# Illumina/strelka

Measured on AMD Instinct MI355X. Metric: candidate-alignment scoring cells/s (read bases x candidate alignments; Strelka2 has no pair-HMM, SURVEY.md section 0) + germline loci/s + 40x WGS-like germline wall-clock (e2e) + 110x/40x somatic wall-clock (e2e_somatic), higher is better.
Workload: dtype f64; 1 GPU; germline chr20-style synthetic (BASELINE.json configs[1]).  Headline: scoreCandidateAlignment as one function -- per GPU per step 65536 reads of 150 bp x 87.9 candidate alignments each (5-7 candidate indels around them), from the candidate alignments the device search left (PCal) to one double each: one kernel (F5: the walk of each alignment's path + the terms of its bases, penalties and clips).  ; read_len=150

## Files before the change

strelka_amd/csrc/read_enumerate.hip:

```cpp

#include "sk_common.h"

#include "align_entry.h"
#include "read_enumerate.h"

#include <algorithm>
#include <chrono>
#include <climits>
#include <cstdio>
#include <cstdlib>
#include <cstring>
#include <vector>

using namespace skcore;

int sk_score_alignments_launch_hostleg(const sk_align_batch* b, double* dev_out_lnp, void* hip_stream);

namespace
{

static_assert(sizeof(PFrame) % 4 == 0 && sizeof(PCal) % 4 == 0, "frames move through LDS as 32-bit words");


struct EnumArgs
// ... 365 lines not shown
    const char* ref;
    int32_t ref_offset, ref_len;
    int32_t n_reads, n_cals;
    const PCal* pool;
    const int32_t* list;
    int32_t* status;
    const int64_t* read_off;
    const uint8_t* read_code;
    const int32_t* cal_off;
    int32_t* win_begin;
    int32_t* win_end;
    int32_t* ins_lo;
    int32_t* ins_hi;
    uint8_t* n_seg8;
    int32_t* win_len;
    int32_t* hap_len;
    int32_t* n_ins;
    int16_t* ins_idx;
    int32_t* ins_off;
    int32_t* n_ops;
    const int64_t* hap_off;
    PCal* cals;
    uint8_t* hap_code;
    const int64_t* op_off;
    sk_score_op* ops;
    uint32_t* entries;
    uint32_t* evmask;
    int32_t evmask_words, max_read_len;
    uint8_t* colmat;
    const int64_t* colmat_off;
    uint32_t* addmask;
    int32_t* ref_outside;
    int32_t n_cals_on_device;
};
enum { INS_CAP = Caps::K + 2 };

__device__ inline int read_of_cal(const FlatArgs& a, const int c)
{
    int lo = 0, hi = a.n_reads;
    while (hi - lo > 1) {
        const int mid = (lo + hi) >> 1;
        if (a.cal_off[mid] <= c) lo = mid; else hi = mid;
    }
    return lo;
}

__global__ __launch_bounds__(256) void pool_bounds_kernel(const FlatArgs a)
{
    const int n_cals = a.n_cals_on_device ? a.cal_off[a.n_reads] : a.n_cals;
    for (int c = blockIdx.x * blockDim.x + threadIdx.x; c < n_cals; c += gridDim.x * blockDim.x) {
    const int r = read_of_cal(a, c);
    const PCal& cal = a.pool[a.list[c]];
    a.n_seg8[c] = uint8_t(min(int(cal.n_seg), 255));
    int32_t wb = INT_MAX, we = INT_MIN, pos = cal.pos;
    for (int i = 0; i < cal.n_seg; ++i) {
        const PSeg s = cal.path[i];
        if (seg_align_match(s.type)) {
            wb = min(wb, pos);
            we = max(we, pos + int32_t(s.length));
            pos += int32_t(s.length);
        } else if (s.type == SK_SEG_DELETE || s.type == SK_SEG_SKIP) {
            pos += int32_t(s.length);
        }
    }
    if (wb <= we) {
        atomicMin(&a.win_begin[r], wb);
        atomicMax(&a.win_end[r], we);
    }
    int lo = INT_MAX, hi = INT_MIN;
    auto add = [&](const int t) {
        if (t < 0 || a.job.tab[t].ins_len == 0) return;
        lo = min(lo, t);
        hi = max(hi, t);
    };
    for (int i = 0; i < cal.n_indels; ++i) add(cal.indels[i]);
    add(cal.lead);
    add(cal.trail);
    if (lo <= hi) {
        atomicMin(&a.ins_lo[r], lo);
        atomicMax(&a.ins_hi[r], hi);
    }
    }
}

__global__ __launch_bounds__(64) void pool_layout_kernel(const FlatArgs a)
{
    const int r = blockIdx.x * blockDim.x + threadIdx.x;
    if (r >= a.n_reads) return;
    const int nc = a.cal_off[r + 1] - a.cal_off[r];
    a.n_ins[r] = 0;
    a.win_len[r] = 0;
    a.hap_len[r] = 0;
    if (nc == 0) return;
    int32_t wb = a.win_begin[r], we = a.win_end[r];
    if (wb > we) wb = we = 0;
    a.win_begin[r] = wb;
    int32_t len = we - wb;
    a.win_len[r] = len;
    int16_t* idx = a.ins_idx + size_t(r) * INS_CAP;
    int32_t* off = a.ins_off + size_t(r) * INS_CAP;
    int n = 0;
    for (int t = a.ins_lo[r]; t <= a.ins_hi[r]; ++t) {
        const uint32_t il = a.job.tab[t].ins_len;
        if (il == 0) continue;
        if (n >= INS_CAP) {
            a.status[r] = ST_OVERFLOW;
            n = 0;
            break;
        }
        idx[n] = int16_t(t);
        off[n] = len;
        len += int32_t(il);
        ++n;
    }
    a.n_ins[r] = n;
    a.hap_len[r] = max(len, 1);
}

__device__ int matching_indel(const PJob& j, const PCal& c, const int32_t ref_head_pos, const unsigned del_len, const unsigned ins_len,
                              const int ends_first, const int ends_second, const int path_index)
{
    if (path_index < ends_first) return c.lead;
    if (path_index > ends_second) return c.trail;
    int found = -1;
    for (int k = 0; k < c.n_indels; ++k) {
        const PIndel& ci = j.tab[c.indels[k]];
        if (ci.pos == ref_head_pos && (ci.type == SK_INDEL_INDEL || ci.type == SK_INDEL_MISMATCH) && ci.del == del_len &&
            ci.ins_len == ins_len) {
            if (found >= 0) return -2;
            found = c.indels[k];
        } else if (ci.pos > ref_head_pos) {
            break;
        }
    }
    return found >= 0 ? found : -2;
}

struct NoOpSink
{
    __device__ __forceinline__ void operator()(uint8_t, uint32_t, int32_t, bool) const {}
};

template <bool WRITE, typename SINK = NoOpSink>
__device__ int flatten_cal(const FlatArgs& a, const int r, const PCal& c, const int32_t read_len, sk_score_op* ops, SINK&& sink = SINK())
{
    const int aps = c.n_seg;
    const int32_t win_begin = a.win_begin[r];
    const int n_ins = a.n_ins[r];
    const int16_t* ins_idx = a.ins_idx + size_t(r) * INS_CAP;
// ... 157 lines not shown
    const int c0 = blockIdx.x * blockDim.x;
    const int c = c0 + lane;
    const int nc = min(64, a.n_cals - c0);
    const int src_k = (lane < nc) ? a.list[c0 + lane] : 0;
    for (int k = 0; k < nc; ++k) {
        const uint32_t* __restrict__ src = reinterpret_cast<const uint32_t*>(a.pool + __shfl(src_k, k));
        uint32_t* __restrict__ dst = reinterpret_cast<uint32_t*>(a.cals + (c0 + k));
        for (int j = lane; j < REC_DW; j += 64) {
            const uint32_t v = src[j];
            s_cal[k * REC_STRIDE + j] = v;
            dst[j] = v;
        }
    }
    __syncthreads();
    if (c >= a.n_cals) return;
    const int r = read_of_cal(a, c);
    const PCal& cal = *reinterpret_cast<const PCal*>(s_cal + lane * REC_STRIDE);
    if (a.status[r] != ST_OK) return;
    (void)flatten_cal<true>(a, r, cal, int32_t(a.read_off[r + 1] - a.read_off[r]), a.ops + a.op_off[c]);
    for (int i = 0; i < cal.n_indels; ++i) (void)job_cand(a.job, cal.indels[i]);
    if (cal.lead >= 0) (void)job_cand(a.job, cal.lead);
    if (cal.trail >= 0) (void)job_cand(a.job, cal.trail);
}

constexpr int F5_MAX_READ = 256;
constexpr int ONE_WAIT_MAX_READS = 16384;
constexpr int F5_MAX_POOL = 768;
#ifndef F5_SORT
#define F5_SORT 1
#endif
constexpr int F5_TAB = 32;

static_assert(F5_TAB <= 64, "the table copy is a lane an entry");

struct FusedScoreArgs
{
    FlatArgs f;
    const uint8_t* read_qual;
    const SkTables* tab;
    double* scores;
    unsigned* err;
    int32_t* n_unhandled;
    int32_t write_cals;
    unsigned long long* dbg;
    unsigned* queue;
};

constexpr int F5_SEGS = 16, F5_INDELS = 8;
constexpr int F5_SLOT = (F5_SEGS + 1) | 1;
__device__ __forceinline__ int f5_ent_word(const int k) { return k; }
constexpr int F5_ROW = 3;

struct F5Tab
{
    int32_t pos;
    uint32_t del, ins_len;
    uint32_t type_cand;
    int32_t ins_at;
};

template <int MAXR>
struct F5Lds
{
    uint8_t read[MAXR + 12];
    uint8_t hap[F5_MAX_POOL + 12];
    double row[(MAXR + 8) * F5_ROW];
// ... 67 lines not shown
        }
    }
    int pi = 0, n_ent = 0;
    int32_t pos = 0, ref_head_pos = c.pos();
    unsigned npen = 0;
    for (;;) {
        const bool live = pi < aps && !bad;
        if (!__any(live)) break;
        const int sh = 4 * (pi & 15);
        const unsigned ty = unsigned(types >> sh) & 15u, ln = seg_len(pi & 15);
        const uint64_t not_run = ~((I4 | D4) >> sh) & N1;
        const int run4 = not_run ? __builtin_ctzll(not_run) : 64;
        const uint64_t run_set = (run4 >= 64) ? ~0ull : ((1ull << run4) - 1ull);
        const bool is_swap = live && ((I4 >> sh) & run_set) != 0ull && ((D4 >> sh) & run_set) != 0ull;
        const bool is_match = (ty == SK_SEG_MATCH || ty == SK_SEG_SEQ_MATCH), is_clip = (ty == SK_SEG_SOFT_CLIP);
        const bool is_indel_seg = is_swap || ty == SK_SEG_SEQ_MISMATCH || ty == SK_SEG_INSERT || ty == SK_SEG_DELETE;
        unsigned del_len = (ty == SK_SEG_INSERT) ? 0u : ln, ins_len = (ty == SK_SEG_DELETE) ? 0u : ln;
        int n_seg = 1;
        unsigned read_step = (is_match || ty == SK_SEG_SEQ_MISMATCH || ty == SK_SEG_INSERT || is_clip) ? ln : 0u;
        unsigned ref_step = (is_match || ty == SK_SEG_SEQ_MISMATCH || ty == SK_SEG_DELETE || ty == SK_SEG_SKIP) ? ln : 0u;
        if (is_swap) {
            n_seg = run4 >> 2;
            del_len = ins_len = 0;
            for (int k = 0; k < n_seg; ++k) {
                const unsigned l = seg_len((pi + k) & 15);
                if ((I4 >> (4 * ((pi + k) & 15))) & 1ull) ins_len += l;
                else del_len += l;
            }
            read_step = ins_len;
            ref_step = del_len;
        }
        const unsigned asked = (del_len << 16) | ins_len;
        const bool askable = del_len < 0xffffu && ins_len < 0xffffu;
        int k_found = 0, n_found = 0;
        bool open = true;
#pragma unroll
        for (int k = 0; k < F5_INDELS; ++k) {
            if (k < ni_wave) {
                const bool m = open && k_pos[k] == ref_head_pos && k_pack[k] == asked;
                k_found = m ? k : k_found;
                n_found += m ? 1 : 0;
                open = open && (m || k_pos[k] <= ref_head_pos);
            }
        }
        int key = (n_found == 1) ? c.indel(k_found) : -2;
        key = (pi < ends_first) ? c.lead() : (pi > ends_second) ? c.trail() : key;
        const bool key_ok = key >= 0;
        const F5Tab te = S.tab[(key_ok ? key : tab_lo) - tab_lo];
        const bool indel_ok = live && is_indel_seg && key_ok;
        if (indel_ok && consulted) consulted[key] = 1;
        const bool pen = is_indel_seg && (te.type_cand >> 8) == 0u;
        const int32_t head = (pi < ends_first) ? int32_t(te.ins_len) - int32_t(ln) : 0;
        const bool ins_bases = is_indel_seg && ins_len > 0u;
        const bool ins_ok = ins_len <= 0xffffu && head >= 0 && uint32_t(head) + ins_len <= te.ins_len && te.ins_at >= 0;
        const bool bases = ins_bases || is_match;
        const int32_t src = ins_bases ? te.ins_at + head : ref_head_pos - win_begin;
        const unsigned len = ins_bases ? ins_len : ln;
        const bool known = is_indel_seg || is_match || is_clip || ty == SK_SEG_SKIP || ty == SK_SEG_HARD_CLIP;
        bool fail = !known || (is_indel_seg && (!key_ok || !askable)) || (ins_bases && !ins_ok);
        const bool entry = (bases || (is_clip && !is_indel_seg)) && len > 0u;
        if (entry) {
            fail = fail || pos + int32_t(len) > L || (bases && (src < 0 || int64_t(src) + int64_t(len) > int64_t(P)));
            const int hidx = bases ? int(src) - pos : 0;
            fail = fail || n_ent > F5_SEGS || npen > 4u || hidx < -256 || hidx > 3839;
            if (live && !fail) myslot[f5_ent_word(n_ent)] = unsigned(pos) | (npen << 9) | (bases ? 0u : 1u << 15) | (unsigned(hidx + 256) << 16);
        }
        if (live) {
            bad = fail;
            n_ent += entry ? 1 : 0;
            npen = entry ? (pen ? 1u : 0u) : npen + (pen ? 1u : 0u);
            pos += int32_t(read_step);
            ref_head_pos += int32_t(ref_step);
            pi += n_seg;
        }
    }
    if (!has) return 0;
    if (bad || pos != L || n_ent > F5_SEGS || npen > 4u) return -1;
    myslot[f5_ent_word(n_ent)] = unsigned(L) | (npen << 9) | (256u << 16);
    return n_ent + 1;
}

template <typename LDS>
__device__ __forceinline__ double f5_sum(LDS& S, const uint32_t* const myslot, const int n_ent, const double ln_noncand, const double ln_quarter)
{
    double lnp = 0.0;
    const unsigned char* rows = reinterpret_cast<const unsigned char*>(S.row);
    int e = 0, p = 0, stop = 0, hidx = 0;
    uint32_t cur = myslot[f5_ent_word(0)], nxt = myslot[f5_ent_word(1)];
    auto next_op = [&]() -> bool {
// ... 42 lines not shown
                uint32_t pm = uint32_t(past >> (32 * h));
                __asm__("" : "+v"(pm));
                sel[h] = (B10 & ~pm & x) | (~B10 & pm);
                __asm__("" : "+v"(sel[h]));
            }
            const unsigned base = __umul24(unsigned(8 * F5_ROW), unsigned(p));
            double v[8];
#pragma unroll
            for (int u = 0; u < 8; ++u) {
                const unsigned at = base + unsigned(8 * F5_ROW * u) + ((sel[u >> 2] >> (8 * (u & 3))) & 0xffu);
                v[u] = *reinterpret_cast<const double*>(rows + at);
            }
#pragma unroll
            for (int u = 0; u < 8; ++u) lnp = __dadd_rn(lnp, v[u]);
            p += mm;
        }
        if (next_op()) break;
    }
    return lnp;
}

__device__ __forceinline__ void f5_wave_sync()
{
    __builtin_amdgcn_fence(__ATOMIC_RELEASE, "workgroup");
    __builtin_amdgcn_wave_barrier();
    __builtin_amdgcn_fence(__ATOMIC_ACQUIRE, "workgroup");
}

template <int MAXR, bool TIMING>
__device__ __forceinline__ void f5_read(const FusedScoreArgs& fa, const int r, F5Lds<MAXR>& S)
{
    auto now = [&]() -> unsigned long long { return TIMING ? (unsigned long long)clock64() : 0ull; };
    const FlatArgs& a = fa.f;
    const int lane = threadIdx.x & 63;
    const int c0 = a.cal_off[r], c1 = a.cal_off[r + 1];
    const int ncr = c1 - c0;
    if (ncr == 0 || a.status[r] != ST_OK) return;
    unsigned long long stamp[8];
    stamp[0] = now();
    const unsigned long long wall0 = TIMING ? (unsigned long long)wall_clock64() : 0ull;
    for (int i = 1; i < 8; ++i) stamp[i] = 0;
    const int64_t ro = a.read_off[r];
    const int32_t L = int32_t(a.read_off[r + 1] - ro);
    const int32_t P = a.hap_len[r];
    if (L > MAXR || P > F5_MAX_POOL) {
        if (lane == 0) atomicAdd(fa.n_unhandled, 1);
        return;
    }
    const int32_t win_begin = a.win_begin[r];
    const int n_ins = a.n_ins[r];
    int my_ins_idx = -1;
    int32_t my_ins_off = 0;
    {
        const int16_t* idx = a.ins_idx + size_t(r) * INS_CAP;
        const int32_t* off = a.ins_off + size_t(r) * INS_CAP;
        int32_t my_ins_len = 0;
        uint32_t my_ins_src = 0;
        if (lane < n_ins) {
            const int t_idx = idx[lane];
            my_ins_idx = t_idx;
            my_ins_off = off[lane];
            my_ins_len = int32_t(a.job.tab[t_idx].ins_len);
            my_ins_src = a.job.tab[t_idx].ins_off;
        }
        const int32_t win_len = a.win_len[r];
        for (int32_t i = lane; i < P + 8; i += 64) {
            uint8_t v = SK_BAM_ANY;
            if (i < win_len) {
                const int32_t p = win_begin + i;
                const bool outside = (p < a.ref_offset || p >= a.ref_offset + a.ref_len);
                if (outside && a.ref_outside) atomicAdd(a.ref_outside, 1);
                v = outside ? uint8_t(SK_BAM_ANY) : code_of(a.ref[p - a.ref_offset]);
            }
            S.hap[i] = v;
        }
        f5_wave_sync();
        for (int k = 0; k < n_ins; ++k) {
            const int32_t o = __builtin_amdgcn_readlane(my_ins_off, k), n = __builtin_amdgcn_readlane(my_ins_len, k);
            const uint32_t src = uint32_t(__builtin_amdgcn_readlane(int(my_ins_src), k));
            for (int32_t i = lane; i < n; i += 64)
                if (o + i < P) S.hap[o + i] = code_of(a.ins_pool[src + uint32_t(i)]);
        }
        const SkTables* __restrict__ T = fa.tab;
        for (int32_t i = lane; i < L + 12; i += 64) {
            unsigned q = 0;
            uint8_t code = SK_BAM_ANY;
            if (i < L) {
                code = a.read_code[ro + i];
                q = fa.read_qual[ro + i];
                if (q > 70u) {
                    atomicOr(fa.err, unsigned(SK_DEVERR_QSCORE));
                    q = 70u;
                }
            }
            S.read[i] = code & 15u;
            if (i < L + 8) {
                const unsigned c = code & 15u;
                const bool adds = i < L && c != 15u;
                const double agree = adds ? T->q2lncompe[q] : 0.0;
                S.row[F5_ROW * i] = agree;
                S.row[F5_ROW * i + 1] = 0.0;
                S.row[F5_ROW * i + 2] = !adds ? 0.0 : (c == 0u) ? agree : T->q2mis[q];
            }
        }
    }
    const double ln_quarter = fa.tab->ln_quarter, ln_noncand = fa.tab->ln_noncand;

    uint8_t* const order = S.hap + ((P + 8 + 3) & ~3);
    const bool sorted_order = (F5_SORT != 0) && ncr > 64 && ncr <= 256 && ((P + 8 + 3) & ~3) + ncr <= int(sizeof(S.hap));
    if (sorted_order) {
        int seg_of[4];
#pragma unroll
        for (int k = 0; k < 4; ++k) {
            const int j = lane + 64 * k;
            seg_of[k] = (j < ncr) ? int(a.n_seg8[c0 + j]) : -1;
            seg_of[k] = min(seg_of[k], F5_SEGS + 1);
        }
        unsigned present = 0;
#pragma unroll
        for (int k = 0; k < 4; ++k) present |= (seg_of[k] >= 0) ? (1u << seg_of[k]) : 0u;
#pragma unroll
        for (int d = 32; d >= 1; d >>= 1) present |= unsigned(__shfl_xor(int(present), d));
        present = unsigned(__builtin_amdgcn_readfirstlane(int(present)));
        int at = 0;
        while (present != 0u) {
            const int v = 31 - __builtin_clz(present);
            present &= ~(1u << v);
#pragma unroll
            for (int k = 0; k < 4; ++k) {
                const uint64_t m = __ballot(seg_of[k] == v);
                if (seg_of[k] == v) order[at + __popcll(m & ((1ull << lane) - 1ull))] = uint8_t(lane + 64 * k);
                at += __popcll(m);
            }
        }
    }
// ... 13 lines not shown
        rec.l0 = rec.l1 = rec.l2 = rec.l3 = 0;
        rec.ind = 0;
        rec.ind_lo = 0;
        uint64_t ind_raw0 = 0, ind_raw1 = 0;
        if (has) {
            const PCal* src = a.pool + a.list[c0 + my_j];
            const uint4* s4 = reinterpret_cast<const uint4*>(src);
            const uint4 q0 = s4[0], q1 = s4[1], q2 = s4[2], q3 = s4[3], q4 = s4[4];
            const uint32_t* si = reinterpret_cast<const uint32_t*>(src->indels);
            const uint32_t i0 = si[0], i1 = si[1], i2 = si[2], i3 = si[3];
            ind_raw0 = uint64_t(i0) | (uint64_t(i1) << 32);
            ind_raw1 = uint64_t(i2) | (uint64_t(i3) << 32);
            rec.w0 = q0.x;
            rec.w1 = q0.y;
            rec.w2 = q0.z;
            const unsigned nseg = (q0.z >> 8) & 0xffu, nind = (q0.z >> 16) & 0xffu;
            fits = (nseg <= unsigned(F5_SEGS) && nind <= unsigned(F5_INDELS));
            uint64_t types = 0;
            bool odd_type = false;
            auto pack4 = [&](const uint32_t a0, const uint32_t a1, const uint32_t a2, const uint32_t a3, const int first) -> uint64_t {
                types |= (uint64_t(a0 & 15u) | (uint64_t(a1 & 15u) << 4) | (uint64_t(a2 & 15u) << 8) | (uint64_t(a3 & 15u) << 12)) << (4 * first);
                odd_type = odd_type || (unsigned(first) < nseg && (a0 & 0xffffu) > 15u) || (unsigned(first + 1) < nseg && (a1 & 0xffffu) > 15u) ||
                           (unsigned(first + 2) < nseg && (a2 & 0xffffu) > 15u) || (unsigned(first + 3) < nseg && (a3 & 0xffffu) > 15u);
                return uint64_t(a0 >> 16) | (uint64_t(a1 >> 16) << 16) | (uint64_t(a2 >> 16) << 32) | (uint64_t(a3 >> 16) << 48);
            };
            rec.l0 = pack4(q0.w, q1.x, q1.y, q1.z, 0);
            rec.l1 = pack4(q1.w, q2.x, q2.y, q2.z, 4);
            rec.l2 = pack4(q2.w, q3.x, q3.y, q3.z, 8);
            rec.l3 = pack4(q3.w, q4.x, q4.y, q4.z, 12);
            rec.types = types;
            fits = fits && !odd_type;
        }
        auto raw_indel = [&](const int k) -> int { return int(int16_t(((k & 4) ? ind_raw1 : ind_raw0) >> (16 * (k & 3)))); };
        int tab_lo = 0;
        {
            int lo = INT_MAX, hi = INT_MIN;
            if (has && fits) {
                auto add = [&](const int i) {
                    lo = min(lo, i);
                    hi = max(hi, i);
                };
                const int ni = rec.n_indels();
                for (int i = 0; i < ni; ++i) add(raw_indel(i));
                if (rec.lead() >= 0) add(rec.lead());
                if (rec.trail() >= 0) add(rec.trail());
            }
#pragma unroll
            for (int d = 32; d > 0; d >>= 1) {
                lo = min(lo, __shfl_xor(lo, d));
                hi = max(hi, __shfl_xor(hi, d));
            }
            const int n_tab = (lo <= hi) ? hi - lo + 1 : 0;
            if (__any(has && !fits) || (n_tab > 0 && lo < 0) || n_tab > F5_TAB) {
                if (lane == 0) atomicAdd(fa.n_unhandled, 1);
                return;
            }
            tab_lo = n_tab ? lo : 0;
            uint64_t ind = 0;
#pragma unroll
            for (int k = 0; k < F5_INDELS; ++k) ind |= uint64_t(unsigned(raw_indel(k) - tab_lo) & 63u) << (6 * k);
            rec.ind = ind;
            rec.ind_lo = tab_lo;
            if (lane < n_tab) {
                const PIndel& g = a.job.tab[tab_lo + lane];
                F5Tab e;
                e.pos = g.pos;
                e.del = g.del;
                e.ins_len = g.ins_len;
                e.type_cand = unsigned(g.type) | (unsigned(g.cand) << 8);
                e.ins_at = -1;
                S.tab[lane] = e;
            }
            f5_wave_sync();
            if (my_ins_idx >= tab_lo && my_ins_idx < tab_lo + n_tab) S.tab[my_ins_idx - tab_lo].ins_at = my_ins_off;
        }
        f5_wave_sync();
        const unsigned long long tc = now();
        stamp[2] += tc - ta;
        int n_ent = 0;
        bool bad = false;
        {
            const unsigned long long tA0 = now();
            n_ent = f5_walk_selects(S, rec, has, tab_lo, win_begin, a.job.consulted, L, P, myslot);
            const unsigned long long tA1 = now();
            stamp[7] += tA1 - tA0;
            bad = n_ent < 0;
            if (has) {
                if (a.job.consulted) {
                    const int ni = rec.n_indels();
                    for (int i = 0; i < ni; ++i) a.job.consulted[rec.indel(i)] = 1;
                    if (rec.lead() >= 0) a.job.consulted[rec.lead()] = 1;
                    if (rec.trail() >= 0) a.job.consulted[rec.trail()] = 1;
                }
                if (bad) a.status[r] = ST_FAIL;
            }
            (void)tA1;
        }
        __builtin_amdgcn_wave_barrier();
        const unsigned long long td = now();
        stamp[4] += td - tc;
        if (has && !bad) {
            const double lnp = f5_sum(S, myslot, n_ent, ln_noncand, ln_quarter);
            fa.scores[c0 + my_j] = lnp;
        }
        stamp[5] += now() - td;
    }
    if (fa.dbg && lane == 0) {
        stamp[6] = now();
        stamp[3] = TIMING ? (unsigned long long)wall_clock64() - wall0 : 0ull;
        for (int i = 0; i < 8; ++i) fa.dbg[size_t(r) * 8 + i] = stamp[i];
    }
}

template <int MAXR, bool TIMING, int WAVES>
__global__ __launch_bounds__(64 * WAVES) __attribute__((amdgpu_waves_per_eu(4, 4))) void flatten_score_kernel(const FusedScoreArgs fa, const int n_reads)
{
    __shared__ __attribute__((aligned(16))) F5Lds<MAXR> S[WAVES];
    const int wave = threadIdx.x >> 6, lane = threadIdx.x & 63;
    for (;;) {
        int r = 0;
        if (lane == 0) r = int(atomicAdd(&fa.queue[0], 1u));
        r = __builtin_amdgcn_readfirstlane(r);
        if (r >= n_reads) break;
        f5_read<MAXR, TIMING>(fa, r, S[wave]);
        f5_wave_sync();
    }
    if (lane == 0) {
// ... 499 lines not shown
    size_t cap = 0;
    int reserve(const size_t bytes)
    {
        if (bytes <= cap) return 0;
        if (p) (void)skrt::hostFree(p);
        p = nullptr;
        cap = 0;
        const size_t want = bytes + bytes / 4 + 4096;
        SK_HIP(skrt::hostMalloc(&p, want));
        cap = want;
        return 0;
    }
    template <typename T> T* as() const { return static_cast<T*>(p); }
};

struct View
{
    void* p = nullptr;
    template <typename T> T* as() const { return static_cast<T*>(p); }
};

struct EnumBuffers
{
    DevBuf in_arena, zero_arena, minmax_arena, mask_arena;
    HostBuf h_in_arena, h_zero_arena;
    View tab, ins, toggle, ref, reads, read_off, read_code, read_qual, r2i, i2r, orig, map_level;
    View counters, status, warn, n_raw, hap_len, fill, n_uniq, consulted;
    View win_begin, ins_lo, win_end, ins_hi, evmask, addmask;
    View h_counters, h_status, h_warn, h_n_raw, h_hap_len, h_n_uniq, h_consulted;
    View cal_off_z, h_cal_off_z;
    DevBuf level_a, level_b, pool, leaf_read, leaf_hash;
    DevBuf raw_off, grouped, ghash, gkey, dup, sorted;
    DevBuf n_ops, win_len, n_ins, ins_idx, ins_off, n_seg8;
    DevBuf cal_off, hap_off, cals, hap_code, op_off, ops, entries, scores, colmat, colmat_off;
    DevBuf s3_order, s3_smooth, s3_flag, s3_rm_type, s3_rm_pos, s3_key, s3_sorted_score, s3_sorted_hash, s3_next_same, s3_range_end, s3_removed, s3_out, s3_list;
    HostBuf h_s3_out, h_s3_list;
    HostBuf h_raw_off, h_n_ops, h_cal_off, h_hap_off, h_op_off, h_cals, h_scores, h_colmat_off;
};
EnumBuffers& bufs()
{
    static EnumBuffers b;
    return b;
}

}

extern "C" int sk_enum_device_available(void) { return sk_ctx().ready ? 1 : 0; }

namespace
{
uint64_t g_generation = 0;
int32_t g_n_cals = 0;
bool g_cals_gathered = false;
const PCal* g_cals_pool = nullptr;
const int32_t* g_cals_list = nullptr;
const double* g_scores = nullptr;

struct LastFlat
{
    bool valid = false;
    bool fused = false;
    FusedScoreArgs fs;
    FlatArgs fa;
    sk_align_batch d;
    int32_t n = 0, n_cals = 0;
    int64_t cells = 0;
// ... 77 lines not shown
                     std::chrono::duration<double, std::milli>(std::chrono::steady_clock::now() - t_begin).count());
    };

    const int64_t n_bases = n ? in->read_off[n] : 0;
    int64_t frame_cap = std::min<int64_t>(std::max<int64_t>(int64_t(n) * 128, 1 << 18), 1 << 23);
    int64_t pool_cap = std::min<int64_t>(std::max<int64_t>(int64_t(n) * 512, 1 << 19), int64_t(32) << 20);
    if (const char* e = std::getenv("SK_ENUM_TEST_CAPS")) {
        long long fc = 0, pc = 0;
        if (std::sscanf(e, "%lld,%lld", &fc, &pc) == 2 && fc > 0 && pc > 0) {
            frame_cap = std::max<int64_t>(fc, n);
            pool_cap = pc;
        }
    }
    bool test_caps = false;
    if (const char* e = std::getenv("SK_ENUM_TEST_CAPS")) test_caps = (e[0] != 0);
    if (one_wait && !test_caps) pool_cap = std::min<int64_t>(pool_cap, std::max<int64_t>(int64_t(n) * 256, 1 << 17));
    const int n_counters = Caps::K + 8 + DYN_COUNT + 2;
#define RES(buf, bytes) \
    if (B.buf.reserve(std::max<size_t>(size_t(bytes), 256))) return 1
#define HRES(buf, bytes) \
    if (B.buf.reserve(size_t(bytes) + 64)) return 1
    RES(level_a, sizeof(PFrame) * size_t(frame_cap));
    RES(level_b, sizeof(PFrame) * size_t(frame_cap));
    RES(pool, sizeof(PCal) * size_t(pool_cap));
    RES(leaf_read, 4 * size_t(pool_cap));
    RES(leaf_hash, 4 * size_t(pool_cap));
    RES(raw_off, 4 * size_t(n + 1));
    RES(win_len, 4 * size_t(n));
    RES(n_ins, 4 * size_t(n));
    RES(ins_idx, 2 * size_t(n) * INS_CAP);
    RES(ins_off, 4 * size_t(n) * INS_CAP);
    RES(cal_off, 4 * size_t(n + 1));
    RES(hap_off, 8 * size_t(n + 1));
    HRES(h_raw_off, 4 * size_t(n + 1));
    HRES(h_cal_off, 4 * size_t(n + 1));
    HRES(h_hap_off, 8 * size_t(n + 1));
    const bool with_stage3 = in->want_scores && in->want_stage3;
    const int W = sk_ent_evmask_words(std::max(in->max_read_len, 0));
    struct Piece
    {
        View* view;
        const void* src;
        size_t bytes, off;
    };
    auto lay_out = [](Piece* pc, const int n_pieces) {
        size_t at = 0;
        for (int i = 0; i < n_pieces; ++i) {
            pc[i].off = at;
            at += (pc[i].bytes + 255) & ~size_t(255);
        }
        return at;
    };
    Piece ins_p[] = {
        { &B.tab, in->tab, sizeof(PIndel) * size_t(in->n_tab), 0 },
        { &B.ins, in->ins_pool, size_t(in->ins_pool_len), 0 },
        { &B.toggle, in->max_toggle, sizeof(uint32_t) * size_t(in->n_max_toggle), 0 },
        { &B.ref, in->ref, size_t(std::max(in->ref_len, 0)), 0 },
        { &B.reads, in->reads, sizeof(PRead) * size_t(n), 0 },
        { &B.read_off, in->read_off, sizeof(int64_t) * size_t(n + 1), 0 },
        { &B.read_code, in->read_code, size_t(n_bases), 0 },
        { &B.read_qual, in->read_qual, size_t(n_bases), 0 },
        { &B.r2i, in->r2i, with_stage3 ? 8 * size_t(in->n_tab) : 0, 0 },
        { &B.i2r, in->i2r, with_stage3 ? 8 * size_t(in->n_tab) : 0, 0 },
        { &B.orig, in->orig, with_stage3 ? 4 * size_t(in->n_tab) : 0, 0 },
        { &B.map_level, in->map_level, with_stage3 ? 4 * size_t(n) : 0, 0 },
    };
// ... 188 lines not shown
        sc.count = B.n_uniq.as<int32_t>();
        sc.off = B.cal_off_z.as<int32_t>();
        sc.list = B.s3_list.as<int32_t>();
        sc.light_cals = light_cals;
        SK_LAUNCH(job_scan_kernel<true>, dim3(1), dim3(1024), 0, st, sc);
        SK_LAUNCH(rank_kernel, dim3(e2_blocks), dim3(256), 0, st, sa);
        FlatArgs fa;
        std::memset(&fa, 0, sizeof(fa));
        fa.job = dj;
        fa.ins_pool = B.ins.as<char>();
        fa.ref = B.ref.as<char>();
        fa.ref_offset = in->ref_offset;
        fa.ref_len = in->ref_len;
        fa.n_reads = n;
        fa.n_cals = n_cap;
        fa.n_cals_on_device = 1;
        fa.pool = ea.pool;
        fa.list = B.sorted.as<int32_t>();
        fa.status = ea.status;
        fa.read_off = B.read_off.as<int64_t>();
        fa.read_code = B.read_code.as<uint8_t>();
        fa.cal_off = B.cal_off_z.as<int32_t>();
        fa.win_begin = B.win_begin.as<int32_t>();
        fa.win_len = B.win_len.as<int32_t>();
        fa.hap_len = B.hap_len.as<int32_t>();
        fa.n_ins = B.n_ins.as<int32_t>();
        fa.ins_idx = B.ins_idx.as<int16_t>();
        fa.ins_off = B.ins_off.as<int32_t>();
        fa.win_end = B.win_end.as<int32_t>();
        fa.ins_lo = B.ins_lo.as<int32_t>();
        fa.ins_hi = B.ins_hi.as<int32_t>();
        fa.n_seg8 = B.n_seg8.as<uint8_t>();
        fa.max_read_len = in->max_read_len;
        fa.ref_outside = dyn + DYN_REF_OUTSIDE;
        SK_LAUNCH(pool_bounds_kernel, dim3(e2_blocks), dim3(256), 0, st, fa);
        SK_LAUNCH(pool_layout_kernel, dim3((n + 63) / 64), dim3(64), 0, st, fa);
        FusedScoreArgs fs;
        fs.f = fa;
        fs.read_qual = B.read_qual.as<uint8_t>();
        fs.tab = ctx.dev_tables;
        fs.scores = B.scores.as<double>();
        fs.err = ctx.dev_error_flags;
        fs.n_unhandled = n_unhandled;
        fs.queue = B.counters.as<unsigned>() + (Caps::K + 8 + DYN_COUNT);
        fs.write_cals = 0;
        fs.dbg = nullptr;
        launch_flatten_score(n, st, fs);
        Stage3Args s3;
        s3.tab.tab = dj.tab;
        s3.tab.r2i = B.r2i.as<double>();
        s3.tab.i2r = B.i2r.as<double>();
        s3.tab.orig = B.orig.as<int32_t>();
        s3.tab.n_tab = in->n_tab;
        s3.tab.max_indel_size = in->max_indel_size;
        s3.tab.consulted = dj.consulted;
        s3.opt = in->stage3_opt;
        s3.n_reads = n;
        s3.status = ea.status;
        s3.cal_off = fa.cal_off;
        s3.cals = fa.pool;
        s3.slot = fa.list;
        s3.scores = B.scores.as<double>();
        s3.read_off = fa.read_off;
        s3.read_code = fa.read_code;
        s3.map_level = B.map_level.as<int32_t>();
        s3.order = B.s3_order.as<int32_t>();
// ... 172 lines not shown

    RES(n_ops, 4 * size_t(n_cals));
    RES(op_off, 8 * size_t(n_cals + 1));
    HRES(h_n_ops, 4 * size_t(n_cals));
    HRES(h_op_off, 8 * size_t(n_cals + 1));
    FlatArgs fa;
    std::memset(&fa, 0, sizeof(fa));
    fa.job = dj;
    fa.ins_pool = B.ins.as<char>();
    fa.ref = B.ref.as<char>();
    fa.ref_offset = in->ref_offset;
    fa.ref_len = in->ref_len;
    fa.n_reads = n;
    fa.n_cals = n_cals;
    fa.pool = ea.pool;
    fa.list = B.sorted.as<int32_t>();
    fa.status = ea.status;
    fa.read_off = B.read_off.as<int64_t>();
    fa.read_code = B.read_code.as<uint8_t>();
    fa.cal_off = B.cal_off.as<int32_t>();
    fa.win_begin = B.win_begin.as<int32_t>();
    fa.win_len = B.win_len.as<int32_t>();
    fa.hap_len = B.hap_len.as<int32_t>();
    fa.n_ins = B.n_ins.as<int32_t>();
    fa.ins_idx = B.ins_idx.as<int16_t>();
    fa.ins_off = B.ins_off.as<int32_t>();
    fa.n_ops = B.n_ops.as<int32_t>();
    fa.win_end = B.win_end.as<int32_t>();
    fa.ins_lo = B.ins_lo.as<int32_t>();
    fa.ins_hi = B.ins_hi.as<int32_t>();
    RES(n_seg8, size_t(n_cals));
    fa.n_seg8 = B.n_seg8.as<uint8_t>();
    fa.ref_outside = B.counters.as<int32_t>() + (Caps::K + 8 + DYN_REF_OUTSIDE);
    SK_HIP(skrt::memsetAsync(B.minmax_arena.p, 0x7f, minmax_p[2].off, st));
    SK_HIP(skrt::memsetAsync(static_cast<char*>(B.minmax_arena.p) + minmax_p[2].off, 0x80, minmax_bytes - minmax_p[2].off, st));
    if (n_cals > 0) SK_LAUNCH(pool_bounds_kernel, dim3((n_cals + 255) / 256), dim3(256), 0, st, fa);
    SK_LAUNCH(pool_layout_kernel, dim3((n + 63) / 64), dim3(64), 0, st, fa);
    SK_HIP(skrt::getLastError());
    const bool fused_enabled = !(std::getenv("SK_A5_FUSED") != nullptr && std::strcmp(std::getenv("SK_A5_FUSED"), "0") == 0);
    const bool try_fused = fused_enabled && in->want_scores && n_cals > 0;
    RES(scores, 8 * size_t(n_cals));
    if (!(in->want_scores && in->want_stage3)) HRES(h_cals, sizeof(PCal) * size_t(n_cals));
    HRES(h_scores, 8 * size_t(n_cals));
    out->cals = B.h_cals.as<PCal>();
    g_n_cals = n_cals;
    fa.max_read_len = in->max_read_len;
    g_cals_pool = fa.pool;
    g_cals_list = fa.list;
    bool cals_in_set_order = false;

    auto after_scores = [&]() -> int {
        D2H(h_scores, scores, 8 * size_t(n_cals));
        out->scores = B.h_scores.as<double>();
        if (in->want_stage3) {
            RES(s3_order, 4 * size_t(n_cals));
            RES(s3_smooth, 8 * size_t(n_cals));
            RES(s3_flag, size_t(n_cals));
            RES(s3_rm_type, size_t(n_bases));
            RES(s3_rm_pos, 4 * size_t(n_bases));
            RES(s3_key, 16 * size_t(n_cals));
            RES(s3_sorted_score, 8 * size_t(n_cals));
            RES(s3_sorted_hash, 4 * size_t(n_cals));
            RES(s3_next_same, 4 * size_t(n_cals));
            RES(s3_removed, size_t(n_cals));
            RES(s3_range_end, 4 * size_t(n_cals));
            RES(s3_out, sizeof(sk3::Out) * size_t(n));
// ... 340 lines not shown
```

Baseline: 758.6 billion cells/s.

## Pre-code reference, pack per-read headers, precompute indel table span for fused scorer

Adds a kernel that pre-encodes the reference into packed 4-byte base codes, so the fused scorer fills each read's haplotype window with aligned word loads and alignbyte instead of per-byte code_of lookups with per-base outside checks. Per-read metadata is packed into a 32-byte header written by the layout kernel, and the pool bounds kernel records each read's indel table span so the scorer can load the table once per read instead of per alignment. It also issues read code and quality loads early into registers, and skips the indel key search when no lane in the wave has an indel segment. The cost is extra buffers, an extra launch over the whole reference, and more registers in the scorer.

Result: slower. 727.0 billion cells/s (-4.2%).

```diff
diff --git a/strelka_amd/csrc/read_enumerate.hip b/strelka_amd/csrc/read_enumerate.hip
--- a/strelka_amd/csrc/read_enumerate.hip
+++ b/strelka_amd/csrc/read_enumerate.hip
@@ -421,8 +421,67 @@
     uint32_t* addmask;
     int32_t* ref_outside;
     int32_t n_cals_on_device;
+    const uint32_t* ref_coded;
+    int32_t ref_coded_words;
+    uint4* read_hdr;
+    int32_t* tab_span;
 };
 enum { INS_CAP = Caps::K + 2 };
+
+constexpr int REF_CODED_PAD = 16;
+__host__ __device__ inline int32_t ref_coded_words_of(const int32_t ref_len) { return (((ref_len > 0 ? ref_len : 0) + 15) & ~15) / 4 + REF_CODED_PAD / 4; }
+
+__global__ __launch_bounds__(256) void ref_code_kernel(const char* __restrict__ ref, const int32_t ref_len, uint32_t* __restrict__ coded )
+{
+    const int n_words = REF_CODED_PAD / 4 + ref_coded_words_of(ref_len);
+    for (int w = blockIdx.x * blockDim.x + threadIdx.x; w < n_words; w += gridDim.x * blockDim.x) {
+        uint32_t v = 0;
+#pragma unroll
+        for (int b = 0; b < 4; ++b) {
+            const int32_t x = 4 * w + b - REF_CODED_PAD;
+            const uint8_t code = (x >= 0 && x < ref_len) ? code_of(ref[x]) : uint8_t(SK_BAM_ANY);
+            v |= uint32_t(code) << (8 * b);
+        }
+        coded[w] = v;
+    }
+}
+
+static int ref_code_blocks(const int32_t ref_len)
+{
+    const int words = REF_CODED_PAD / 4 + ref_coded_words_of(ref_len);
+    return std::max(1, std::min((words + 255) / 256, 1024));
+}
+
+struct ReadHdr
+{
+    int32_t c0, ncr;
+    int64_t read_off;
+    int32_t win_begin;
+    uint32_t win_hap;
+    uint32_t tab_span;
+    uint32_t len_ins_st;
+};
+constexpr uint32_t READ_HDR_NO_SPAN = 0xffffffffu;
+constexpr int F5_TAB_SPAN = 32;
+constexpr uint32_t READ_HDR_NOT_OK = 1u << 24;
+static_assert(sizeof(ReadHdr) == 32, "two 16-byte words");
+static_assert(INS_CAP <= 255, "a byte in the header");
+
+__device__ inline void write_read_hdr(const FlatArgs& a, const int r)
+{
+    const int64_t ro = a.read_off[r];
+    const int64_t len = a.read_off[r + 1] - ro;
+    const int32_t c0 = a.cal_off[r];
+    const uint32_t w7 = uint32_t(len < 0 || len > 0xffff ? 0xffff : len) | (uint32_t(a.n_ins[r]) << 16) | (a.status[r] != ST_OK ? READ_HDR_NOT_OK : 0u);
+    a.read_hdr[2 * size_t(r)] = make_uint4(uint32_t(c0), uint32_t(a.cal_off[r + 1] - c0), uint32_t(uint64_t(ro)), uint32_t(uint64_t(ro) >> 32));
+    const int32_t wl = a.win_len[r], hl = a.hap_len[r];
+    const uint32_t w5 = uint32_t(wl < 0 || wl > 0xffff ? 0xffff : wl) | (uint32_t(hl < 0 || hl > 0xffff ? 0xffff : hl) << 16);
+    const int32_t t_lo = a.tab_span[2 * size_t(r)], t_hi = -a.tab_span[2 * size_t(r) + 1];
+    uint32_t w6 = READ_HDR_NO_SPAN;
+    if (t_lo > t_hi) w6 = 0u;
+    else if (t_lo >= 0 && t_lo <= 0xffff && t_hi - t_lo + 1 <= F5_TAB_SPAN) w6 = uint32_t(t_lo) | (uint32_t(t_hi - t_lo + 1) << 16);
+    a.read_hdr[2 * size_t(r) + 1] = make_uint4(uint32_t(a.win_begin[r]), w5, w6, w7);
+}
 
 __device__ inline int read_of_cal(const FlatArgs& a, const int c)
 {
@@ -469,6 +528,23 @@
         atomicMin(&a.ins_lo[r], lo);
         atomicMax(&a.ins_hi[r], hi);
     }
+    int t_lo = INT_MAX, t_hi = INT_MIN;
+    for (int i = 0; i < cal.n_indels; ++i) {
+        t_lo = min(t_lo, int(cal.indels[i]));
+        t_hi = max(t_hi, int(cal.indels[i]));
+    }
+    if (cal.lead >= 0) {
+        t_lo = min(t_lo, int(cal.lead));
+        t_hi = max(t_hi, int(cal.lead));
+    }
+    if (cal.trail >= 0) {
+        t_lo = min(t_lo, int(cal.trail));
+        t_hi = max(t_hi, int(cal.trail));
+    }
+    if (t_lo <= t_hi) {
+        atomicMin(&a.tab_span[2 * size_t(r)], t_lo);
+        atomicMin(&a.tab_span[2 * size_t(r) + 1], -t_hi);
+    }
     }
 }
 
@@ -480,7 +556,10 @@
     a.n_ins[r] = 0;
     a.win_len[r] = 0;
     a.hap_len[r] = 0;
-    if (nc == 0) return;
+    if (nc == 0) {
+        write_read_hdr(a, r);
+        return;
+    }
     int32_t wb = a.win_begin[r], we = a.win_end[r];
     if (wb > we) wb = we = 0;
     a.win_begin[r] = wb;
@@ -504,6 +583,7 @@
     }
     a.n_ins[r] = n;
     a.hap_len[r] = max(len, 1);
+    write_read_hdr(a, r);
 }
 
 __device__ int matching_indel(const PJob& j, const PCal& c, const int32_t ref_head_pos, const unsigned del_len, const unsigned ins_len,
@@ -727,6 +807,7 @@
 constexpr int F5_TAB = 32;
 
 static_assert(F5_TAB <= 64, "the table copy is a lane an entry");
+static_assert(F5_TAB == F5_TAB_SPAN, "the span pool_layout_kernel accepts is the table copy's");
 
 struct FusedScoreArgs
 {
@@ -860,29 +941,35 @@
         }
         const unsigned asked = (del_len << 16) | ins_len;
         const bool askable = del_len < 0xffffu && ins_len < 0xffffu;
-        int k_found = 0, n_found = 0;
-        bool open = true;
+        bool key_ok = false, pen = false;
+        int32_t ins_src = 0;
+        bool ins_ok = false;
+        if (__builtin_amdgcn_ballot_w64(live && is_indel_seg) != 0ull) {
+            int k_found = 0, n_found = 0;
+            bool open = true;
 #pragma unroll
-        for (int k = 0; k < F5_INDELS; ++k) {
-            if (k < ni_wave) {
-                const bool m = open && k_pos[k] == ref_head_pos && k_pack[k] == asked;
-                k_found = m ? k : k_found;
-                n_found += m ? 1 : 0;
-                open = open && (m || k_pos[k] <= ref_head_pos);
-            }
-        }
-        int key = (n_found == 1) ? c.indel(k_found) : -2;
-        key = (pi < ends_first) ? c.lead() : (pi > ends_second) ? c.trail() : key;
-        const bool key_ok = key >= 0;
-        const F5Tab te = S.tab[(key_ok ? key : tab_lo) - tab_lo];
-        const bool indel_ok = live && is_indel_seg && key_ok;
-        if (indel_ok && consulted) consulted[key] = 1;
-        const bool pen = is_indel_seg && (te.type_cand >> 8) == 0u;
-        const int32_t head = (pi < ends_first) ? int32_t(te.ins_len) - int32_t(ln) : 0;
+            for (int k = 0; k < F5_INDELS; ++k) {
+                if (k < ni_wave) {
+                    const bool m = open && k_pos[k] == ref_head_pos && k_pack[k] == asked;
+                    k_found = m ? k : k_found;
+                    n_found += m ? 1 : 0;
+                    open = open && (m || k_pos[k] <= ref_head_pos);
+                }
+            }
+            int key = (n_found == 1) ? c.indel(k_found) : -2;
+            key = (pi < ends_first) ? c.lead() : (pi > ends_second) ? c.trail() : key;
+            key_ok = key >= 0;
+            const F5Tab te = S.tab[(key_ok ? key : tab_lo) - tab_lo];
+            const bool indel_ok = live && is_indel_seg && key_ok;
+            if (indel_ok && consulted) consulted[key] = 1;
+            pen = is_indel_seg && (te.type_cand >> 8) == 0u;
+            const int32_t head = (pi < ends_first) ? int32_t(te.ins_len) - int32_t(ln) : 0;
+            ins_ok = ins_len <= 0xffffu && head >= 0 && uint32_t(head) + ins_len <= te.ins_len && te.ins_at >= 0;
+            ins_src = te.ins_at + head;
+        }
         const bool ins_bases = is_indel_seg && ins_len > 0u;
-        const bool ins_ok = ins_len <= 0xffffu && head >= 0 && uint32_t(head) + ins_len <= te.ins_len && te.ins_at >= 0;
         const bool bases = ins_bases || is_match;
-        const int32_t src = ins_bases ? te.ins_at + head : ref_head_pos - win_begin;
+        const int32_t src = ins_bases ? ins_src : ref_head_pos - win_begin;
         const unsigned len = ins_bases ? ins_len : ln;
         const bool known = is_indel_seg || is_match || is_clip || ty == SK_SEG_SKIP || ty == SK_SEG_HARD_CLIP;
         bool fail = !known || (is_indel_seg && (!key_ok || !askable)) || (ins_bases && !ins_ok);
@@ -991,28 +1078,41 @@
 {
     auto now = [&]() -> unsigned long long { return TIMING ? (unsigned long long)clock64() : 0ull; };
     const FlatArgs& a = fa.f;
-    const int lane = threadIdx.x & 63;
-    const int c0 = a.cal_off[r], c1 = a.cal_off[r + 1];
-    const int ncr = c1 - c0;
-    if (ncr == 0 || a.status[r] != ST_OK) return;
+    int lane = threadIdx.x & 63;
+    __asm__("" : "+v"(lane));
+    const uint4 h0 = a.read_hdr[2 * size_t(r)], h1 = a.read_hdr[2 * size_t(r) + 1];
+    const int c0 = int(h0.x), ncr = int(h0.y);
+    if (ncr == 0 || (h1.w & READ_HDR_NOT_OK) != 0u) return;
     unsigned long long stamp[8];
     stamp[0] = now();
     const unsigned long long wall0 = TIMING ? (unsigned long long)wall_clock64() : 0ull;
     for (int i = 1; i < 8; ++i) stamp[i] = 0;
-    const int64_t ro = a.read_off[r];
-    const int32_t L = int32_t(a.read_off[r + 1] - ro);
-    const int32_t P = a.hap_len[r];
+    const int64_t ro = int64_t(uint64_t(h0.z) | (uint64_t(h0.w) << 32));
+    const int32_t L = int32_t(h1.w & 0xffffu);
+    const int32_t P = int32_t(h1.y >> 16);
     if (L > MAXR || P > F5_MAX_POOL) {
         if (lane == 0) atomicAdd(fa.n_unhandled, 1);
         return;
     }
-    const int32_t win_begin = a.win_begin[r];
-    const int n_ins = a.n_ins[r];
+    const int32_t win_begin = int32_t(h1.x);
+    const int n_ins = int((h1.w >> 16) & 0xffu);
     int my_ins_idx = -1;
     int32_t my_ins_off = 0;
+    const bool read_tab = h1.z != READ_HDR_NO_SPAN;
+    const int rt_lo = read_tab ? int(h1.z & 0xffffu) : 0, rt_n = read_tab ? int(h1.z >> 16) : 0;
     {
         const int16_t* idx = a.ins_idx + size_t(r) * INS_CAP;
         const int32_t* off = a.ins_off + size_t(r) * INS_CAP;
+        constexpr int ROW_IT = (MAXR + 12 + 63) / 64;
+        uint8_t rd_code[ROW_IT], rd_qual[ROW_IT];
+#pragma unroll
+        for (int k = 0; k < ROW_IT; ++k) {
+            const int32_t i = lane + 64 * k;
+            const int32_t ic = max(min(i, L - 1), 0);
+            const uint8_t code = a.read_code[ro + ic], qual = fa.read_qual[ro + ic];
+            rd_code[k] = (i < L) ? code : uint8_t(SK_BAM_ANY);
+            rd_qual[k] = (i < L) ? qual : uint8_t(0);
+        }
         int32_t my_ins_len = 0;
         uint32_t my_ins_src = 0;
         if (lane < n_ins) {
@@ -1022,18 +1122,57 @@
             my_ins_len = int32_t(a.job.tab[t_idx].ins_len);
             my_ins_src = a.job.tab[t_idx].ins_off;
         }
-        const int32_t win_len = a.win_len[r];
-        for (int32_t i = lane; i < P + 8; i += 64) {
-            uint8_t v = SK_BAM_ANY;
-            if (i < win_len) {
-                const int32_t p = win_begin + i;
-                const bool outside = (p < a.ref_offset || p >= a.ref_offset + a.ref_len);
-                if (outside && a.ref_outside) atomicAdd(a.ref_outside, 1);
-                v = outside ? uint8_t(SK_BAM_ANY) : code_of(a.ref[p - a.ref_offset]);
-            }
-            S.hap[i] = v;
+        const int32_t win_len = int32_t(h1.y & 0xffffu);
+        if (lane < rt_n) {
+            const PIndel& g = a.job.tab[rt_lo + lane];
+            F5Tab e;
+            e.pos = g.pos;
+            e.del = g.del;
+            e.ins_len = g.ins_len;
+            e.type_cand = unsigned(g.type) | (unsigned(g.cand) << 8);
+            e.ins_at = -1;
+            S.tab[lane] = e;
+        }
+        {
+            const int32_t x0 = win_begin - a.ref_offset;
+            const int32_t w0 = x0 >> 2;
+            const uint32_t* const cw = a.ref_coded;
+            const int32_t w_lo = -(REF_CODED_PAD / 4), w_hi = a.ref_coded_words;
+            constexpr uint32_t ANY4 = 0x01010101u * uint32_t(SK_BAM_ANY);
+            constexpr int WIN_IT = (F5_MAX_POOL + 8 + 3) / 4 / 64 + 1;
+            static_assert(WIN_IT * 64 * 4 >= F5_MAX_POOL + 8, "the window copy covers the pool and its pad");
+            const int32_t n_words = (P + 8 + 3) >> 2;
+            uint32_t lo[WIN_IT], hi[WIN_IT];
+#pragma unroll
+            for (int k = 0; k < WIN_IT; ++k) {
+                const int32_t j = lane + 64 * k;
+                const int64_t w = int64_t(w0) + j;
+                const bool need = j < n_words && 4 * j < win_len;
+                const bool ok_lo = need && w >= w_lo && w < w_hi, ok_hi = need && w + 1 >= w_lo && w + 1 < w_hi;
+                const int64_t wc_lo = max(min(w, int64_t(w_hi) - 1), int64_t(w_lo)), wc_hi = max(min(w + 1, int64_t(w_hi) - 1), int64_t(w_lo));
+                const uint32_t v_lo = cw[wc_lo], v_hi = cw[wc_hi];
+                lo[k] = ok_lo ? v_lo : ANY4;
+                hi[k] = ok_hi ? v_hi : ANY4;
+            }
+#pragma unroll
+            for (int k = 0; k < WIN_IT; ++k) {
+                const int32_t j = lane + 64 * k;
+                if (j < n_words) {
+                    uint32_t v = __builtin_amdgcn_alignbyte(hi[k], lo[k], unsigned(x0) & 3u);
+                    const int32_t keep = win_len - 4 * j;
+                    const uint32_t m = (keep >= 4) ? 0xffffffffu : (keep <= 0) ? 0u : ((1u << (8 * keep)) - 1u);
+                    v = (v & m) | (ANY4 & ~m);
+                    *reinterpret_cast<uint32_t*>(S.hap + 4 * j) = v;
+                }
+            }
+            if (a.ref_outside && lane == 0) {
+                const int64_t b = max(int64_t(x0), int64_t(0)), e = min(int64_t(x0) + win_len, int64_t(a.ref_len));
+                const int32_t outside = win_len - int32_t(max(e - b, int64_t(0)));
+                if (outside > 0) atomicAdd(a.ref_outside, outside);
+            }
         }
         f5_wave_sync();
+        if (my_ins_idx >= rt_lo && my_ins_idx < rt_lo + rt_n) S.tab[my_ins_idx - rt_lo].ins_at = my_ins_off;
         for (int k = 0; k < n_ins; ++k) {
             const int32_t o = __builtin_amdgcn_readlane(my_ins_off, k), n = __builtin_amdgcn_readlane(my_ins_len, k);
             const uint32_t src = uint32_t(__builtin_amdgcn_readlane(int(my_ins_src), k));
@@ -1041,25 +1180,30 @@
                 if (o + i < P) S.hap[o + i] = code_of(a.ins_pool[src + uint32_t(i)]);
         }
         const SkTables* __restrict__ T = fa.tab;
-        for (int32_t i = lane; i < L + 12; i += 64) {
-            unsigned q = 0;
-            uint8_t code = SK_BAM_ANY;
-            if (i < L) {
-                code = a.read_code[ro + i];
-                q = fa.read_qual[ro + i];
-                if (q > 70u) {
-                    atomicOr(fa.err, unsigned(SK_DEVERR_QSCORE));
-                    q = 70u;
+        double agree[ROW_IT], differ[ROW_IT];
+#pragma unroll
+        for (int k = 0; k < ROW_IT; ++k) {
+            const int32_t i = lane + 64 * k;
+            unsigned q = rd_qual[k];
+            if (q > 70u) {
+                atomicOr(fa.err, unsigned(SK_DEVERR_QSCORE));
+                q = 70u;
+            }
+            const unsigned c = rd_code[k] & 15u;
+            const bool adds = i < L && c != 15u;
+            agree[k] = adds ? T->q2lncompe[q] : 0.0;
+            differ[k] = !adds ? 0.0 : (c == 0u) ? agree[k] : T->q2mis[q];
+        }
+#pragma unroll
+        for (int k = 0; k < ROW_IT; ++k) {
+            const int32_t i = lane + 64 * k;
+            if (i < L + 12) {
+                S.read[i] = rd_code[k] & 15u;
+                if (i < L + 8) {
+                    S.row[F5_ROW * i] = agree[k];
+                    S.row[F5_ROW * i + 1] = 0.0;
+                    S.row[F5_ROW * i + 2] = differ[k];
                 }
-            }
-            S.read[i] = code & 15u;
-            if (i < L + 8) {
-                const unsigned c = code & 15u;
-                const bool adds = i < L && c != 15u;
-                const double agree = adds ? T->q2lncompe[q] : 0.0;
-                S.row[F5_ROW * i] = agree;
-                S.row[F5_ROW * i + 1] = 0.0;
-                S.row[F5_ROW * i + 2] = !adds ? 0.0 : (c == 0u) ? agree : T->q2mis[q];
             }
         }
     }
@@ -1139,8 +1283,18 @@
             fits = fits && !odd_type;
         }
         auto raw_indel = [&](const int k) -> int { return int(int16_t(((k & 4) ? ind_raw1 : ind_raw0) >> (16 * (k & 3)))); };
-        int tab_lo = 0;
-        {
+        int tab_lo = rt_lo;
+        if (read_tab) {
+            if (__any(has && !fits)) {
+                if (lane == 0) atomicAdd(fa.n_unhandled, 1);
+                return;
+            }
+            uint64_t ind = 0;
+#pragma unroll
+            for (int k = 0; k < F5_INDELS; ++k) ind |= uint64_t(unsigned(raw_indel(k) - tab_lo) & 63u) << (6 * k);
+            rec.ind = ind;
+            rec.ind_lo = tab_lo;
+        } else {
             int lo = INT_MAX, hi = INT_MIN;
             if (has && fits) {
                 auto add = [&](const int i) {
@@ -1199,7 +1353,10 @@
                     if (rec.lead() >= 0) a.job.consulted[rec.lead()] = 1;
                     if (rec.trail() >= 0) a.job.consulted[rec.trail()] = 1;
                 }
-                if (bad) a.status[r] = ST_FAIL;
+                if (bad) {
+                    a.status[r] = ST_FAIL;
+                    atomicOr(&a.read_hdr[2 * size_t(r) + 1].w, READ_HDR_NOT_OK);
+                }
             }
             (void)tA1;
         }
@@ -1765,6 +1922,7 @@
     DevBuf level_a, level_b, pool, leaf_read, leaf_hash;
     DevBuf raw_off, grouped, ghash, gkey, dup, sorted;
     DevBuf n_ops, win_len, n_ins, ins_idx, ins_off, n_seg8;
+    DevBuf ref_coded, read_hdr, tab_span;
     DevBuf cal_off, hap_off, cals, hap_code, op_off, ops, entries, scores, colmat, colmat_off;
     DevBuf s3_order, s3_smooth, s3_flag, s3_rm_type, s3_rm_pos, s3_key, s3_sorted_score, s3_sorted_hash, s3_next_same, s3_range_end, s3_removed, s3_out, s3_list;
     HostBuf h_s3_out, h_s3_list;
@@ -1908,6 +2066,9 @@
     RES(ins_off, 4 * size_t(n) * INS_CAP);
     RES(cal_off, 4 * size_t(n + 1));
     RES(hap_off, 8 * size_t(n + 1));
+    RES(ref_coded, REF_CODED_PAD + 4 * size_t(ref_coded_words_of(in->ref_len)));
+    RES(read_hdr, sizeof(ReadHdr) * size_t(n));
+    RES(tab_span, 8 * size_t(n));
     HRES(h_raw_off, 4 * size_t(n + 1));
     HRES(h_cal_off, 4 * size_t(n + 1));
     HRES(h_hap_off, 8 * size_t(n + 1));
@@ -2162,6 +2323,12 @@
         fa.ins_hi = B.ins_hi.as<int32_t>();
         fa.n_seg8 = B.n_seg8.as<uint8_t>();
         fa.max_read_len = in->max_read_len;
+        fa.ref_coded = B.ref_coded.as<uint32_t>() + REF_CODED_PAD / 4;
+        fa.ref_coded_words = ref_coded_words_of(in->ref_len);
+        fa.read_hdr = B.read_hdr.as<uint4>();
+        fa.tab_span = B.tab_span.as<int32_t>();
+        SK_HIP(skrt::memsetAsync(B.tab_span.p, 0x7f, 8 * size_t(n), st));
+        SK_LAUNCH(ref_code_kernel, dim3(ref_code_blocks(in->ref_len)), dim3(256), 0, st, fa.ref, fa.ref_len, B.ref_coded.as<uint32_t>());
         fa.ref_outside = dyn + DYN_REF_OUTSIDE;
         SK_LAUNCH(pool_bounds_kernel, dim3(e2_blocks), dim3(256), 0, st, fa);
         SK_LAUNCH(pool_layout_kernel, dim3((n + 63) / 64), dim3(64), 0, st, fa);
@@ -2400,6 +2567,13 @@
     RES(n_seg8, size_t(n_cals));
     fa.n_seg8 = B.n_seg8.as<uint8_t>();
     fa.ref_outside = B.counters.as<int32_t>() + (Caps::K + 8 + DYN_REF_OUTSIDE);
+    fa.ref_coded = B.ref_coded.as<uint32_t>() + REF_CODED_PAD / 4;
+    fa.ref_coded_words = ref_coded_words_of(in->ref_len);
+    fa.read_hdr = B.read_hdr.as<uint4>();
+    fa.tab_span = B.tab_span.as<int32_t>();
+    SK_HIP(skrt::memsetAsync(B.tab_span.p, 0x7f, 8 * size_t(n), st));
+    if (in->want_scores && !(std::getenv("SK_A5_FUSED") != nullptr && std::strcmp(std::getenv("SK_A5_FUSED"), "0") == 0))
+        SK_LAUNCH(ref_code_kernel, dim3(ref_code_blocks(in->ref_len)), dim3(256), 0, st, fa.ref, fa.ref_len, B.ref_coded.as<uint32_t>());
     SK_HIP(skrt::memsetAsync(B.minmax_arena.p, 0x7f, minmax_p[2].off, st));
     SK_HIP(skrt::memsetAsync(static_cast<char*>(B.minmax_arena.p) + minmax_p[2].off, 0x80, minmax_bytes - minmax_p[2].off, st));
     if (n_cals > 0) SK_LAUNCH(pool_bounds_kernel, dim3((n_cals + 255) / 256), dim3(256), 0, st, fa);
```
